# highlando/dolfin_navier_scipy

Measured on NVIDIA B200. Metric: cylinder-wake DoF*steps/s, higher is better.
Workload: dtype f64

## Files before the change

dolfin_navier_scipy_b200/csrc/dnsb_api.cu:

```cuda
#include "../../include/dnsb.h"

#include <algorithm>
#include <cmath>
#include <cstdlib>
#include <cstring>
#include <ctime>
#include <new>

#include "dnsb_common.cuh"
#include <cuda.h>
#ifdef DNSB_NO_NC
#define __restrict__
#endif
#include "dnsb_kernels.cuh"
#include "dnsb_batched.cuh"
#include "dnsb_dense.cuh"
#include "dnsb_stream.cuh"
#include "dnsb_tc.cuh"
#include "dnsb_tile.cuh"

#define DNSB_VERSION 100

#define LAUNCH(ctx, kern, grid, block, smem, ...)                              \
  do {                                                                         \
// ... 307 lines not shown
  DNSB_CK(ctx, m->t_runs.upload(runs.data(), runs.size(), ctx->stream));
  DNSB_CK(ctx, m->t_pidx.upload(pidx.data(), pidx.size(), ctx->stream));
  DNSB_CK(ctx, m->t_pval.upload(pval.data(), pval.size(), ctx->stream));
  {
    std::vector<float> pvalf(pval.size());
    std::vector<int> pidxf(pidx.size());
    for (size_t q = 0; q < pval.size(); ++q) pvalf[q] = (float)pval[q];
    for (size_t q = 0; q < pidx.size(); ++q) pidxf[q] = pidx[q] / 2;
    DNSB_CK(ctx, m->t_pvalf.upload(pvalf.data(), pvalf.size(), ctx->stream));
    DNSB_CK(ctx, m->t_pidxf.upload(pidxf.data(), pidxf.size(), ctx->stream));
  }
  p.ok = true;
  return 0;
}

static void csr_free(dnsb_csr *m) {
  if (!m) return;
  m->t_uptr.release(); m->t_rptr.release(); m->t_runs.release(); m->t_pidx.release(); m->t_pval.release();
  m->t_pidxf.release(); m->t_pvalf.release(); m->t_truns.release(); m->t_tdesc.release(); m->t_pdesc.release();
  m->indptr.release(); m->indices.release(); m->v1.release(); m->v2.release();
  delete m;
}

static inline bool batched_ok(const dnsb_csr *A, int nb) {
  return nb > 1 && (size_t)std::max(A->ncols, A->nrows) * nb < ((size_t)1 << 31);
}

static int g_rows_per_cta = 4;
static int g_dense_ctas_per_sm = 2;
static int g_graphs = 1;
static int g_schur_tf32 = 0;
static int g_dmma = 1;
static int g_schur_l2keep = 0;
static int g_tc_ctas = 1;
static int g_schur_tc = 1;
static const int TC_SMEM_OPTIN = 208 * 1024;
static int g_conv_colours = 0;
static inline int spb_gpc(dnsb_ctx *ctx, int nrows, int nb) {
  const long total = (long)nrows * nb;
  long gpc = std::max<long>(1, ((long)g_rows_per_cta * nb) / SPB_THREADS);
  const long groups = (total + SPB_THREADS - 1) / SPB_THREADS;
  while (gpc > 1 && (groups + gpc - 1) / gpc < 2L * ctx->sm_count) gpc /= 2;
  return (int)gpc;
}
static int g_pair = 1;
static inline bool pair_ok(const dnsb_csr *A, int nb) {
  return g_pair && batched_ok(A, nb) && nb % 2 == 0;
}
static inline unsigned spb2_grid(int nrows, int nb) {
  return cdiv((size_t)nrows * (nb / 2), SPB_THREADS);
}
static int g_rowpair = 1;
static inline int rowpairs_of(const dnsb_csr *A, int nb) {
  return (g_rowpair && pair_ok(A, nb)) ? A->npair_rows / 2 : 0;
}
static inline unsigned spp_grid(int npairs, int nb) {
  return cdiv((size_t)npairs * (nb / 2), SPB_THREADS);
}
#define D2C(p) reinterpret_cast<const double2 *>(p)
#define D2(p) reinterpret_cast<double2 *>(p)
static inline unsigned spb_grid(int nrows, int nb, int gpc) {
  return cdiv((size_t)nrows * nb, (size_t)SPB_THREADS * gpc);
}

static int g_tma_min_rows = 65536;
static inline bool spt_ok(const dnsb_csr *A, int nb) {
  return nb == 1 && A->spt.stages >= 2 && A->nrows >= g_tma_min_rows;
// ... 82 lines not shown
    const size_t threads = (size_t)A->nrows * nb;
    LAUNCH(ctx, k_spmm<1>, cdiv(threads, 256), 256, 0, A->view(), coef, x, z, y,
           nb, alpha, beta);
  }
}

static void fill_tabulation(double phi[7][6], double dphi[7][6][3], double qw[7], double lam[7][3]) {
  const double s15 = std::sqrt(15.0);
  const double a1 = (6.0 - s15) / 21.0, a2 = (6.0 + s15) / 21.0;
  const double w1 = (155.0 - s15) / 1200.0, w2 = (155.0 + s15) / 1200.0;
  const double qp[7][3] = {{1. / 3, 1. / 3, 1. / 3},
                           {1 - 2 * a1, a1, a1}, {a1, 1 - 2 * a1, a1}, {a1, a1, 1 - 2 * a1},
                           {1 - 2 * a2, a2, a2}, {a2, 1 - 2 * a2, a2}, {a2, a2, 1 - 2 * a2}};
  const double w[7] = {9. / 40, w1, w1, w1, w2, w2, w2};
  for (int q = 0; q < 7; ++q) {
    const double l0 = qp[q][0], l1 = qp[q][1], l2 = qp[q][2];
    qw[q] = w[q];
    lam[q][0] = l0; lam[q][1] = l1; lam[q][2] = l2;
    phi[q][0] = l0 * (2 * l0 - 1); phi[q][1] = l1 * (2 * l1 - 1);
    phi[q][2] = l2 * (2 * l2 - 1); phi[q][3] = 4 * l1 * l2;
    phi[q][4] = 4 * l0 * l2;       phi[q][5] = 4 * l0 * l1;
    for (int a = 0; a < 6; ++a)
      for (int i = 0; i < 3; ++i) dphi[q][a][i] = 0.0;
    dphi[q][0][0] = 4 * l0 - 1; dphi[q][1][1] = 4 * l1 - 1; dphi[q][2][2] = 4 * l2 - 1;
    dphi[q][3][1] = 4 * l2; dphi[q][3][2] = 4 * l1;
    dphi[q][4][0] = 4 * l2; dphi[q][4][2] = 4 * l0;
    dphi[q][5][0] = 4 * l1; dphi[q][5][1] = 4 * l0;
  }
}

#define DNSB_SWITCH_LIST(X) X(g_rows_per_cta) X(g_pair) X(g_tma_min_rows) X(g_gs_tma) X(g_tma_rows) X(g_tma_stages) \
  X(g_dmma) X(g_schur_tf32) X(g_schur_tc) X(g_tile) X(g_gs_pyth) X(g_schur_l2keep) X(g_tile_stages)             \
  X(g_tile_stages_f) X(g_tail_warps) X(g_pkeep) X(g_proj_t) X(g_cheb_f32) X(g_conv_colours) X(g_rowpair)         \
  X(g_graphs) X(g_dense_ctas_per_sm) X(g_tilef_ctas) X(g_tc_ctas) X(g_init_tile)
static void switches_store(int *sw) {
  int k = 0;
#define X(name) sw[k++] = name;
  DNSB_SWITCH_LIST(X)
#undef X
}
static void switches_load(const int *sw) {
  int k = 0;
#define X(name) name = sw[k++];
  DNSB_SWITCH_LIST(X)
#undef X
}
static const dnsb_ctx *g_switch_owner = nullptr;
static inline cudaError_t dnsb_enter(const dnsb_ctx *ctx) {
  if (g_switch_owner != ctx) { switches_load(ctx->sw); g_switch_owner = ctx; }
  return cudaSetDevice(ctx->device);
}

extern "C" int dnsb_version(void) { return DNSB_VERSION; }

extern "C" int dnsb_ctx_create(int device, dnsb_ctx **out) {
  if (!out) return -2;
  *out = nullptr;
  dnsb_ctx *ctx = new (std::nothrow) dnsb_ctx();
  if (!ctx) return -3;
  ctx->device = device;
  {
    static int defaults[32];
    static bool have_defaults = false;
    if (!have_defaults) { switches_store(defaults); have_defaults = true; }
    switches_load(defaults);
  }
  if (const char *ev = getenv("DNSB_ROWS_PER_CTA")) g_rows_per_cta = std::max(1, atoi(ev));
  if (const char *ev = getenv("DNSB_PAIR")) g_pair = atoi(ev);
  if (const char *ev = getenv("DNSB_TMA_MIN_ROWS")) g_tma_min_rows = atoi(ev);
  if (const char *ev = getenv("DNSB_GS_TMA")) g_gs_tma = atoi(ev);
  if (const char *ev = getenv("DNSB_TMA_ROWS")) g_tma_rows = std::min(SPT_ROWS, std::max(4, atoi(ev) & ~3));
  if (const char *ev = getenv("DNSB_TMA_STAGES")) g_tma_stages = std::min(SPT_MAX_STAGES, std::max(2, atoi(ev)));
  if (const char *ev = getenv("DNSB_DMMA")) g_dmma = atoi(ev);
  if (const char *ev = getenv("DNSB_SCHUR_TF32")) g_schur_tf32 = atoi(ev);
  if (const char *ev = getenv("DNSB_SCHUR_TC")) g_schur_tc = atoi(ev);
  if (const char *ev = getenv("DNSB_TILE")) g_tile = atoi(ev);
  if (const char *ev = getenv("DNSB_GS_PYTH")) g_gs_pyth = atoi(ev);
  if (const char *ev = getenv("DNSB_INIT_TILE")) g_init_tile = atoi(ev);
  if (const char *ev = getenv("DNSB_TC_CTAS")) g_tc_ctas = atoi(ev);
  if (const char *ev = getenv("DNSB_TILEF_CTAS")) g_tilef_ctas = atoi(ev);
  if (const char *ev = getenv("DNSB_PDL")) ctx->pdl = atoi(ev);
  if (const char *ev = getenv("DNSB_PDL_ONLY")) ctx->pdl_only = ev;
  if (const char *ev = getenv("DNSB_PDL_SKIP")) ctx->pdl_skip = ev;
  if (const char *ev = getenv("DNSB_SCHUR_L2KEEP")) g_schur_l2keep = atoi(ev);
  if (const char *ev = getenv("DNSB_TILE_STAGES")) g_tile_stages = std::max(2, std::min(TILE_MAX_STAGES, atoi(ev)));
  if (const char *ev = getenv("DNSB_TILE_STAGES_F")) g_tile_stages_f = std::max(2, std::min(TILE_MAX_STAGES, atoi(ev)));
  if (const char *ev = getenv("DNSB_TAIL_WARPS")) g_tail_warps = std::max(0, std::min(TILE_TAIL_WARPS_MAX, atoi(ev)));
  if (const char *ev = getenv("DNSB_PKEEP")) g_pkeep = atoi(ev);
  if (const char *ev = getenv("DNSB_PROJ_T")) g_proj_t = atoi(ev);
  if (const char *ev = getenv("DNSB_CHEB_F32")) g_cheb_f32 = atoi(ev);
  if (const char *ev = getenv("DNSB_CONV_COLOURS")) g_conv_colours = atoi(ev);
  if (const char *ev = getenv("DNSB_ROWPAIR")) g_rowpair = atoi(ev);
  if (const char *ev = getenv("DNSB_GRAPHS")) g_graphs = atoi(ev);
  if (const char *ev = getenv("DNSB_DENSE_CTAS_PER_SM")) g_dense_ctas_per_sm = std::max(1, atoi(ev));
  switches_store(ctx->sw);
  g_switch_owner = ctx;
  *out = ctx;
  DNSB_CK(ctx, cudaSetDevice(device));
  cudaDeviceProp prop;
  DNSB_CK(ctx, cudaGetDeviceProperties(&prop, device));
  ctx->sm_count = prop.multiProcessorCount;
  ctx->cc = prop.major * 10 + prop.minor;
  ctx->mem_bytes = prop.totalGlobalMem;
  DNSB_CK(ctx, cudaStreamCreateWithFlags(&ctx->stream, cudaStreamNonBlocking));
  double phi[7][6], dphi[7][6][3], qw[7], lam[7][3];
  fill_tabulation(phi, dphi, qw, lam);
  DNSB_CK(ctx, cudaMemcpyToSymbol(c_phi, phi, sizeof phi));
  DNSB_CK(ctx, cudaMemcpyToSymbol(c_dphi, dphi, sizeof dphi));
  DNSB_CK(ctx, cudaMemcpyToSymbol(c_qw, qw, sizeof qw));
  DNSB_CK(ctx, cudaMemcpyToSymbol(c_lam, lam, sizeof lam));
  DNSB_CK(ctx, cudaFuncSetAttribute(k_mdot_b, cudaFuncAttributeMaxDynamicSharedMemorySize, 200 * 1024));
  DNSB_CK(ctx, cudaFuncSetAttribute(k_gs_tma<false>, cudaFuncAttributeMaxDynamicSharedMemorySize, 112 * 1024));
// ... 610 lines not shown
  DNSB_CK(ctx, s->gg.alloc((size_t)(mr + 1) * nb));
  DNSB_CK(ctx, s->gh.alloc((size_t)(mr + 2) * nb));
  DNSB_CK(ctx, s->gh2.alloc((size_t)(mr + 2) * nb));
  DNSB_CK(ctx, s->ginvh.alloc(nb));
  DNSB_CK(ctx, s->gbnorm.alloc(nb));
  DNSB_CK(ctx, s->gresid.alloc(nb));
  DNSB_CK(ctx, s->gdone.alloc(nb));
  DNSB_CK(ctx, s->gits.alloc(nb));
  DNSB_CK(ctx, s->gittot.alloc(nb));
  DNSB_CK(ctx, s->gflags.alloc(4));
  DNSB_CK(ctx, s->grelmax.alloc(nb));
  DNSB_CK(ctx, s->grelmax.zero(ctx->stream));
  s->gs.R = s->gR.p; s->gs.cs = s->gcs.p; s->gs.sn = s->gsn.p; s->gs.g = s->gg.p;
  s->gs.h = s->gh.p; s->gs.invh = s->ginvh.p; s->gs.bnorm = s->gbnorm.p;
  s->gs.resid = s->gresid.p; s->gs.done = s->gdone.p; s->gs.its = s->gits.p;
  s->gs.ittot = s->gittot.p; s->gs.flags = s->gflags.p; s->gs.relmax = s->grelmax.p; s->gs.mr = mr;
  DNSB_CK(ctx, cudaMallocHost((void **)&s->h_flags, 4 * sizeof(int)));
  DNSB_CK(ctx, cudaStreamSynchronize(ctx->stream));
  DNSB_CK(ctx, cudaGetLastError());
  return 0;
}

static void dense_split(dnsb_ctx *ctx, int n, int nb, int *tn, DenseSplit *sp) {
  *tn = nb <= 16 ? 16 : (nb <= 32 ? 32 : 64);
  const int rt = cdiv(n, DGK_TM);
  sp->ksteps = cdiv(n, DGK_TK);
  const long units = (long)rt * sp->ksteps;
  long P = std::min<long>(units, (long)g_dense_ctas_per_sm * ctx->sm_count);
  sp->upc = (int)((units + P - 1) / P);
  sp->nctas = (int)((units + sp->upc - 1) / sp->upc);
  sp->maxseg = 2 + sp->upc / sp->ksteps;
}

typedef CUresult (*dnsb_encode_tiled_fn)(CUtensorMap *, CUtensorMapDataType, cuuint32_t, void *,
                                         const cuuint64_t *, const cuuint64_t *, const cuuint32_t *,
                                         const cuuint32_t *, CUtensorMapInterleave, CUtensorMapSwizzle,
                                         CUtensorMapL2promotion, CUtensorMapFloatOOBfill);
static dnsb_encode_tiled_fn tc_encode_fn() {
  static dnsb_encode_tiled_fn fn = nullptr;
  if (!fn) {
    void *p = nullptr;
    cudaDriverEntryPointQueryResult q;
    if (cudaGetDriverEntryPoint("cuTensorMapEncodeTiled", &p, cudaEnableDefault, &q) == cudaSuccess &&
        q == cudaDriverEntryPointSuccess)
      fn = (dnsb_encode_tiled_fn)p;
  }
  return fn;
}
static bool tc_map_2d(CUtensorMap *map, const float *base, int rows, int cols, int ld, int box_rows) {
  dnsb_encode_tiled_fn enc = tc_encode_fn();
  if (!enc) return false;
  const cuuint64_t gdim[2] = {(cuuint64_t)cols, (cuuint64_t)rows};
  const cuuint64_t gstride[1] = {(cuuint64_t)ld * sizeof(float)};
  const cuuint32_t box[2] = {TC_BK, (cuuint32_t)box_rows};
  const cuuint32_t estr[2] = {1, 1};
  return enc(map, CU_TENSOR_MAP_DATA_TYPE_FLOAT32, 2, (void *)base, gdim, gstride, box, estr,
             CU_TENSOR_MAP_INTERLEAVE_NONE, CU_TENSOR_MAP_SWIZZLE_128B, CU_TENSOR_MAP_L2_PROMOTION_L2_256B,
             CU_TENSOR_MAP_FLOAT_OOB_FILL_NONE) == CUDA_SUCCESS;
}
static cudaError_t tc_setup(dnsb_ctx *ctx, MgLevel *L, int n, int nb) {
  TcPlan &p = L->tc;
  p.ok = false;
  if (ctx->cc < 100 || nb < 8 || nb > 256 || n < TC_BM) return cudaSuccess;
  p.np_ = (nb + 15) & ~15;
  p.kblocks = (n + TC_BK - 1) / TC_BK;
  p.mtiles = (n + TC_BM - 1) / TC_BM;
  const int per_sm = std::max(1, std::min(2, g_tc_ctas));
  p.splits = std::max(1, std::min(p.kblocks, per_sm * ctx->sm_count / p.mtiles));
  p.kb_per_split = (p.kblocks + p.splits - 1) / p.splits;
  p.splits = (p.kblocks + p.kb_per_split - 1) / p.kb_per_split;
  const size_t a_bytes = (size_t)TC_BM * TC_BK * 4;
  const size_t b_bytes = (((size_t)p.np_ * TC_BK * 4) + 1023) & ~(size_t)1023;
  p.stages = (int)std::min<size_t>(TC_MAX_STAGES, ((size_t)TC_SMEM_OPTIN / per_sm - 1024) / (a_bytes + b_bytes));
  if (p.stages < 2) return cudaSuccess;
  p.smem = (size_t)p.stages * (a_bytes + b_bytes) + 1024;
  p.ldx = (n + 3) & ~3;
  cudaError_t e;
  if ((e = L->xt.alloc((size_t)p.np_ * p.ldx)) != cudaSuccess) return e;
  if ((e = L->xt.zero(ctx->stream)) != cudaSuccess) return e;
  if ((e = L->tcpart.alloc((size_t)p.splits * p.mtiles * TC_BM * p.np_)) != cudaSuccess) return e;
  if ((e = L->dinv_f32.alloc((size_t)p.mtiles * p.kblocks * TC_BM * TC_BK)) != cudaSuccess) return e;
  LAUNCH(ctx, k_tc_pack_d, cdiv(L->dinv_f32.n, 256), 256, 0, (const double *)L->dinv_dense.p, L->dinv_f32.p, n,
         p.mtiles, p.kblocks);
  p.ok = tc_map_2d(&p.mapB, L->xt.p, p.np_, n, p.ldx, p.np_);
  return cudaSuccess;
}

static void level_free(MgLevel *L) {
  if (!L) return;
  L->dinv_dense.release(); L->gpart.release(); L->dinv_f32.release(); L->x_f32.release(); L->xt.release(); L->tcpart.release(); L->dinv_own.release(); L->b.release(); L->x.release();
  L->r.release(); L->d0.release(); L->d1.release(); L->t.release();
  delete L;
}

extern "C" void dnsb_solver_destroy(dnsb_solver *s) {
  if (!s) return;
  dnsb_enter(s->ctx);
  const bool trace = getenv("DNSB_TRACE_DESTROY") != nullptr;
  auto now = [] { timespec ts; clock_gettime(CLOCK_MONOTONIC, &ts); return ts.tv_sec + 1e-9 * ts.tv_nsec; };
  double t0 = now();
  auto lap = [&](const char *what) { if (trace) { double t = now(); fprintf(stderr, "[destroy] %-12s %.2f ms\n", what, 1e3 * (t - t0)); t0 = t; } };
  cudaStreamSynchronize(s->ctx->stream);
  lap("sync");
  for (cudaGraphExec_t g : s->igraph) if (g) cudaGraphExecDestroy(g);
  s->igraph.clear();
  lap("graphs");
  csr_free(s->K);
  lap("K");
  s->coef.release(); s->dinv.release(); s->diagpos.release();
  s->Vb.release(); s->Zb.release(); s->w.release();
  lap("bases");
  s->cf_res.release(); s->cf_d0.release(); s->cf_d1.release(); s->cf_z.release(); s->cf_dinv.release();
  s->cres.release(); s->cd0.release(); s->cd1.release();
  s->partial.release(); s->partial2.release(); s->red.release();
  s->gR.release(); s->gcs.release(); s->gsn.release(); s->gg.release(); s->gh.release(); s->gh2.release();
  s->ginvh.release(); s->gbnorm.release(); s->gresid.release(); s->grelmax.release();
  s->gdone.release(); s->gits.release(); s->gittot.release(); s->gflags.release();
// ... 123 lines not shown
  dnsb_ctx *ctx = s->ctx;
  DNSB_REQUIRE(ctx, mp_dinv && mp_scale, "null arguments");
  DNSB_CK(ctx, dnsb_enter(ctx));
  DNSB_CK(ctx, s->mp_dinv.upload(mp_dinv, s->np, ctx->stream));
  DNSB_CK(ctx, s->mp_scale.upload(mp_scale, s->nb, ctx->stream));
  s->has_mass = true;
  solver_drop_graphs(s);
  return 0;
}

extern "C" int dnsb_solver_set_schur_lsc(dnsb_solver *s, const double *du_inv) {
  if (!s) return -2;
  dnsb_ctx *ctx = s->ctx;
  DNSB_REQUIRE(ctx, du_inv != nullptr, "null argument");
  DNSB_REQUIRE(ctx, !s->levels.empty(), "add the levels of L = J Du^-1 JT first");
  DNSB_CK(ctx, dnsb_enter(ctx));
  const size_t nvb = (size_t)s->nv * s->nb, npb = (size_t)s->np * s->nb;
  DNSB_CK(ctx, s->lsc_dinv.upload(du_inv, s->nv, ctx->stream));
  DNSB_CK(ctx, s->lsc_t1.alloc(nvb)); DNSB_CK(ctx, s->lsc_t2.alloc(nvb));
  DNSB_CK(ctx, s->lsc_p1.alloc(npb)); DNSB_CK(ctx, s->lsc_p2.alloc(npb));
  s->has_lsc = true;
  solver_drop_graphs(s);
  return 0;
}

static int dense_apply(dnsb_solver *s, MgLevel *L, const double *x,
                       double *y, double alpha, bool with_mass) {
  dnsb_ctx *ctx = s->ctx;
  const int n = L->n, nb = s->nb;
  const double *ad = with_mass ? s->mp_dinv.p : nullptr;
  const double *as = with_mass ? s->mp_scale.p : nullptr;
  if (L->tc.ok) {
    const TcPlan &p = L->tc;
    int tmem_cols = 32;
    while (tmem_cols < p.np_) tmem_cols *= 2;
    LAUNCH(ctx, k_tc_pack_x, dim3(cdiv(p.ldx, 32), cdiv(nb, 32)), 256, 0, x, L->xt.p, n, nb, p.ldx);
    LAUNCH(ctx, k_schur_tc, dim3(p.mtiles, p.splits), TC_THREADS, p.smem, (const float *)L->dinv_f32.p, p.mapB, L->tcpart.p, p.np_,
           p.kblocks, p.kb_per_split, p.stages, tmem_cols, g_schur_l2keep);
    LAUNCH(ctx, k_tc_epilogue, cdiv((size_t)n * nb, 256), 256, 0, (const float *)L->tcpart.p, p.splits,
           (size_t)p.mtiles * TC_BM * p.np_, p.np_, x, y, n, nb, alpha, ad, as);
    return 0;
  }
  if (nb <= 1)
    LAUNCH(ctx, k_dense_gemv<1>, cdiv((size_t)n * 32, 256), 256, 0, L->dinv_dense.p, x, y, n, nb, alpha, ad, as);
  else if (nb <= 2)
    LAUNCH(ctx, k_dense_gemv<2>, cdiv((size_t)n * 32, 256), 256, 0, L->dinv_dense.p, x, y, n, nb, alpha, ad, as);
  else if (nb <= 4)
    LAUNCH(ctx, k_dense_gemv<4>, cdiv((size_t)n * 32, 256), 256, 0, L->dinv_dense.p, x, y, n, nb, alpha, ad, as);
  else if (nb <= 8)
    LAUNCH(ctx, k_dense_gemv<8>, cdiv((size_t)n * 32, 256), 256, 0, L->dinv_dense.p, x, y, n, nb, alpha, ad, as);
  else {
    int tn;
    DenseSplit sp;
    dense_split(ctx, n, nb, &tn, &sp);
    const dim3 grid(sp.nctas, cdiv(nb, tn));
    if (g_schur_tf32 && L->dinv_f32.p && L->x_f32.p && tn == 64) {
      LAUNCH(ctx, k_f64_to_f32, cdiv((size_t)n * nb, 256), 256, 0, x, L->x_f32.p, (size_t)n, (size_t)nb, (size_t)nb);
const float *df_ = L->dinv_f32.p, *xf_ = L->x_f32.p;
      if (g_schur_tf32 == 1)
        LAUNCH(ctx, k_dense_tf32_streamk<3>, grid, 128, TFM_SMEM_BYTES, df_, L->ldf, xf_, L->gpart.p, n, nb, sp);
      else if (g_schur_tf32 == 2)
        LAUNCH(ctx, k_dense_tf32_streamk<2>, grid, 128, TFM_SMEM_BYTES, df_, L->ldf, xf_, L->gpart.p, n, nb, sp);
      else
        LAUNCH(ctx, k_dense_tf32_streamk<1>, grid, 128, TFM_SMEM_BYTES, df_, L->ldf, xf_, L->gpart.p, n, nb, sp);
    } else if (g_dmma && nb > 32 && n % 2 == 0 && nb % 2 == 0)
      LAUNCH(ctx, k_dense_dmma_streamk, grid, 128, DMM_SMEM_BYTES, L->dinv_dense.p, x, L->gpart.p, n, nb, sp);
    else if (tn == 16)
      LAUNCH(ctx, k_dense_gemm_streamk<16>, grid, 128, 0, L->dinv_dense.p, x, L->gpart.p, n, nb, sp);
    else if (tn == 32)
      LAUNCH(ctx, k_dense_gemm_streamk<32>, grid, 128, 0, L->dinv_dense.p, x, L->gpart.p, n, nb, sp);
    else
      LAUNCH(ctx, k_dense_gemm_streamk<64>, grid, 128, 0, L->dinv_dense.p, x, L->gpart.p, n, nb, sp);
    LAUNCH(ctx, k_dense_epilogue, cdiv((size_t)n * nb, 256), 256, 0, (const double *)L->gpart.p, sp, x,
// ... 1919 lines not shown
```

dolfin_navier_scipy_b200/csrc/dnsb_tc.cuh:

```cuda
#pragma once
#include <cuda.h>
#include <cuda_runtime.h>
#include <cstdint>

#define TC_BM 128
#define TC_BK 32
#define TC_UK 8
#define TC_THREADS 192
#define TC_MAX_STAGES 8

struct TcPlan {
  CUtensorMap mapB;
  int np_ = 0;
  int mtiles = 0, splits = 0, kblocks = 0, kb_per_split = 0, stages = 0;
  int ldx = 0;
  size_t smem = 0;
  bool ok = false;
};

__device__ __forceinline__ uint32_t tc_smem(const void *p) {
  return (uint32_t)__cvta_generic_to_shared(p);
}
__device__ __forceinline__ void tc_mbar_init(uint64_t *b, uint32_t count) {
  asm volatile("mbarrier.init.shared::cta.b64 [%0], %1;" ::"r"(tc_smem(b)), "r"(count) : "memory");
}
__device__ __forceinline__ void tc_mbar_expect(uint64_t *b, uint32_t bytes) {
  asm volatile("mbarrier.arrive.expect_tx.shared::cta.b64 _, [%0], %1;" ::"r"(tc_smem(b)), "r"(bytes)
               : "memory");
}
__device__ __forceinline__ void tc_mbar_wait(uint64_t *b, uint32_t parity) {
  const uint32_t a = tc_smem(b);
  uint32_t ok;
  do {
    asm volatile(
        "{\n\t.reg .pred p;\n\t"
        "mbarrier.try_wait.parity.shared::cta.b64 p, [%1], %2;\n\t"
        "selp.u32 %0, 1, 0, p;\n\t}"
        : "=r"(ok)
        : "r"(a), "r"(parity)
        : "memory");
  } while (!ok);
}
__device__ __forceinline__ void tc_tma_2d(void *dst, const CUtensorMap *map, int c0, int c1, uint64_t *bar) {
  asm volatile(
      "cp.async.bulk.tensor.2d.shared::cluster.global.mbarrier::complete_tx::bytes [%0], [%1, {%2, %3}], [%4];"
      ::"r"(tc_smem(dst)), "l"(map), "r"(c0), "r"(c1), "r"(tc_smem(bar))
      : "memory");
}
__device__ __forceinline__ uint64_t tc_desc(uint32_t saddr) {
  uint64_t d = 0;
  d |= (uint64_t)((saddr >> 4) & 0x3FFF);
  d |= (uint64_t)1 << 16;
  d |= (uint64_t)(1024 >> 4) << 32;
  d |= (uint64_t)1 << 46;
  d |= (uint64_t)2 << 61;
  return d;
}
__device__ __forceinline__ void tc_mma_tf32(uint32_t tmem_d, uint64_t da, uint64_t db, uint32_t idesc,
                                            uint32_t accumulate) {
  asm volatile(
      "{\n\t.reg .pred p;\n\t"
      "setp.ne.b32 p, %4, 0;\n\t"
      "tcgen05.mma.cta_group::1.kind::tf32 [%0], %1, %2, %3, p;\n\t}"
      ::"r"(tmem_d), "l"(da), "l"(db), "r"(idesc), "r"(accumulate)
      : "memory");
}
__device__ __forceinline__ void tc_commit(uint64_t *bar) {
  asm volatile("tcgen05.commit.cta_group::1.mbarrier::arrive::one.shared::cluster.b64 [%0];" ::"r"(tc_smem(bar))
               : "memory");
}
__device__ __forceinline__ void tc_ld16(uint32_t taddr, uint32_t (&r)[16]) {
  asm volatile(
      "tcgen05.ld.sync.aligned.32x32b.x16.b32 "
      "{%0, %1, %2, %3, %4, %5, %6, %7, %8, %9, %10, %11, %12, %13, %14, %15}, [%16];"
      : "=r"(r[0]), "=r"(r[1]), "=r"(r[2]), "=r"(r[3]), "=r"(r[4]), "=r"(r[5]), "=r"(r[6]), "=r"(r[7]),
        "=r"(r[8]), "=r"(r[9]), "=r"(r[10]), "=r"(r[11]), "=r"(r[12]), "=r"(r[13]), "=r"(r[14]), "=r"(r[15])
      : "r"(taddr)
      : "memory");
}

__device__ __forceinline__ void tc_bulk_1d(void *dst, const void *src, uint32_t bytes, uint64_t *bar) {
  asm volatile("cp.async.bulk.shared::cluster.global.mbarrier::complete_tx::bytes [%0], [%1], %2, [%3];" ::"r"(
                   tc_smem(dst)),
               "l"(src), "r"(bytes), "r"(tc_smem(bar))
               : "memory");
}

__global__ void __launch_bounds__(TC_THREADS, 1)
k_schur_tc(const float *__restrict__ Dt, const __grid_constant__ CUtensorMap mapB,
           float *__restrict__ part, int NP, int kblocks, int kb_per_split, int stages, int tmem_cols,
           int l2keep) {
  extern __shared__ __align__(1024) unsigned char tc_raw[];
  __shared__ __align__(8) uint64_t full[TC_MAX_STAGES], empty[TC_MAX_STAGES], accum_full;
  __shared__ uint32_t tmem_base_s;
  unsigned char *ring = (unsigned char *)(((uintptr_t)tc_raw + 1023) & ~(uintptr_t)1023);
  const uint32_t a_bytes = TC_BM * TC_BK * 4, b_bytes = (uint32_t)NP * TC_BK * 4;
  const uint32_t stage_bytes = a_bytes + ((b_bytes + 1023) & ~1023u);
  const int warp = threadIdx.x >> 5, lane = threadIdx.x & 31;
  const int mtile = blockIdx.x, split = blockIdx.y;
  const int kb0 = split * kb_per_split, kb1 = min(kblocks, kb0 + kb_per_split);
  const int nkb = kb1 - kb0;

  if (threadIdx.x == 0) {
    for (int s = 0; s < stages; ++s) {
      tc_mbar_init(&full[s], 1);
      tc_mbar_init(&empty[s], 1);
    }
    tc_mbar_init(&accum_full, 1);
    asm volatile("fence.mbarrier_init.release.cluster;" ::: "memory");
    asm volatile("fence.proxy.async.shared::cta;" ::: "memory");
  }
  if (warp == 1) {
    asm volatile("tcgen05.alloc.cta_group::1.sync.aligned.shared::cta.b32 [%0], %1;" ::"r"(tc_smem(&tmem_base_s)),
                 "r"((uint32_t)tmem_cols)
                 : "memory");
    asm volatile("tcgen05.relinquish_alloc_permit.cta_group::1.sync.aligned;" ::: "memory");
  }
  asm volatile("tcgen05.fence::before_thread_sync;" ::: "memory");
  __syncthreads();
  asm volatile("tcgen05.fence::after_thread_sync;" ::: "memory");
  const uint32_t tmem_base = tmem_base_s;
  dnsb_pdl_entry();

  if (warp == 0) {
    if (lane == 0) {
      for (int i = 0; i < nkb; ++i) {
        const int s = i % stages;
        if (i >= stages) tc_mbar_wait(&empty[s], ((i / stages) - 1) & 1);
        unsigned char *st = ring + (size_t)s * stage_bytes;
        tc_mbar_expect(&full[s], a_bytes + b_bytes);
        tc_bulk_1d(st, Dt + ((size_t)mtile * kblocks + kb0 + i) * (TC_BM * TC_BK), a_bytes, &full[s]);
        tc_tma_2d(st + a_bytes, &mapB, (kb0 + i) * TC_BK, 0, &full[s]);
      }
    }
  } else if (warp == 1) {
    const uint32_t idesc = (1u << 4) | (2u << 7) | (2u << 10) | ((uint32_t)(NP >> 3) << 17) |
                           ((uint32_t)(TC_BM >> 4) << 24);
    for (int i = 0; i < nkb; ++i) {
      const int s = i % stages;
      tc_mbar_wait(&full[s], (i / stages) & 1);
      asm volatile("tcgen05.fence::after_thread_sync;" ::: "memory");
      if (lane == 0) {
        const uint32_t sa = tc_smem(ring + (size_t)s * stage_bytes), sb = sa + a_bytes;
        const uint64_t da = tc_desc(sa), db = tc_desc(sb);
#pragma unroll
        for (int k = 0; k < TC_BK / TC_UK; ++k)
          tc_mma_tf32(tmem_base, da + (uint64_t)(k * 2), db + (uint64_t)(k * 2), idesc, (i | k) != 0);
        tc_commit(&empty[s]);
        if (i == nkb - 1) tc_commit(&accum_full);
      }
      __syncwarp();
    }
  } else {
    const int q = warp & 3;
    const int row = mtile * TC_BM + q * 32 + lane;
    float *out = part + ((size_t)split * gridDim.x * TC_BM + row) * NP;
    if (nkb > 0) {
      tc_mbar_wait(&accum_full, 0);
      asm volatile("tcgen05.fence::after_thread_sync;" ::: "memory");
      for (int c = 0; c < NP; c += 16) {
        uint32_t r[16];
        tc_ld16(tmem_base + ((uint32_t)(q * 32) << 16) + (uint32_t)c, r);
        asm volatile("tcgen05.wait::ld.sync.aligned;" ::: "memory");
        float4 *o4 = reinterpret_cast<float4 *>(out + c);
#pragma unroll
        for (int v = 0; v < 4; ++v)
          o4[v] = make_float4(__uint_as_float(r[4 * v]), __uint_as_float(r[4 * v + 1]),
                              __uint_as_float(r[4 * v + 2]), __uint_as_float(r[4 * v + 3]));
      }
    } else {
      for (int c = 0; c < NP; ++c) out[c] = 0.0f;
    }
  }
  asm volatile("tcgen05.fence::before_thread_sync;" ::: "memory");
  __syncthreads();
  if (warp == 1)
    asm volatile("tcgen05.dealloc.cta_group::1.sync.aligned.b32 %0, %1;" ::"r"(tmem_base), "r"((uint32_t)tmem_cols)
                 : "memory");
}

__device__ __forceinline__ float tc_round_tf32(float v) {
  uint32_t r;
  asm("cvt.rna.tf32.f32 %0, %1;" : "=r"(r) : "f"(v));
  return __uint_as_float(r);
}

__global__ void k_tc_pack_d(const double *__restrict__ src, float *__restrict__ dst, int n, int mtiles,
                            int kblocks) {
  dnsb_pdl_entry();
  const size_t t = (size_t)blockIdx.x * blockDim.x + threadIdx.x;
  const size_t total = (size_t)mtiles * kblocks * TC_BM * TC_BK;
  if (t >= total) return;
  const int k = (int)(t & 31), r = (int)((t >> 5) & 127);
  const size_t tile = t >> 12;
  const int kb = (int)(tile % kblocks), mt = (int)(tile / kblocks);
  const int row = mt * TC_BM + r, col = kb * TC_BK + k;
  const float v = (row < n && col < n) ? tc_round_tf32((float)src[(size_t)row * n + col]) : 0.0f;
  dst[tile * (TC_BM * TC_BK) + (size_t)r * 32 + ((((k >> 2) ^ (r & 7)) << 2) | (k & 3))] = v;
}

__global__ void k_tc_pack_x(const double *__restrict__ x, float *__restrict__ xt, int n, int nb, int ldx) {
  dnsb_pdl_entry();
  __shared__ float tile[32][33];
  const int k0 = blockIdx.x * 32, m0 = blockIdx.y * 32;
  const int tx = threadIdx.x & 31, ty = threadIdx.x >> 5;
  for (int r = ty; r < 32; r += 8) {
    const int k = k0 + r, m = m0 + tx;
    tile[r][tx] = (k < n && m < nb) ? tc_round_tf32((float)x[(size_t)k * nb + m]) : 0.0f;
  }
  __syncthreads();
  for (int r = ty; r < 32; r += 8) {
    const int m = m0 + r, k = k0 + tx;
    if (m < nb && k < ldx) xt[(size_t)m * ldx + k] = tile[tx][r];
  }
}

__global__ void k_tc_epilogue(const float *__restrict__ part, int splits, size_t split_stride, int NP,
                              const double *__restrict__ x, double *__restrict__ y, int n, int nb,
                              double alpha, const double *__restrict__ add_dinv,
                              const double *__restrict__ add_scale) {
  dnsb_pdl_entry();
  const size_t t = (size_t)blockIdx.x * blockDim.x + threadIdx.x;
  if (t >= (size_t)n * nb) return;
  const int i = (int)(t / nb), m = (int)(t % nb);
  double v = 0.0;
  for (int s = 0; s < splits; ++s) v += (double)part[(size_t)s * split_stride + (size_t)i * NP + m];
  if (add_dinv) v += add_scale[m] * add_dinv[i] * x[t];
  y[t] = alpha * v;
}
```

Baseline: 1.771 billion.

## Stream-K split for tcgen05 Schur GEMM with double-buffered TMEM accumulators

Replaces the fixed split-K grid of the TF32 tcgen05 Schur-complement GEMM with a stream-K partition, so each CTA processes a contiguous range of (mtile, kblock) units across tile boundaries. The output is written to per-segment slots, and the epilogue reduces over exactly the slots covering each tile. Two TMEM accumulators let the MMA warp start the next segment while the store warps drain the previous one. The A-operand loads are issued before the PDL wait so they overlap the previous kernel. The B operand is now packed by a new kernel into swizzled per-kblock blocks loaded with 1D bulk copies, which drops the tensor-map TMA path. The cost is a more complex kernel, extra partial slots to reduce, and a grid-stride epilogue.

```diff
diff --git a/dolfin_navier_scipy_b200/csrc/dnsb_api.cu b/dolfin_navier_scipy_b200/csrc/dnsb_api.cu
--- a/dolfin_navier_scipy_b200/csrc/dnsb_api.cu
+++ b/dolfin_navier_scipy_b200/csrc/dnsb_api.cu
@@ -363,7 +363,8 @@
 static int g_schur_tf32 = 0;
 static int g_dmma = 1;
 static int g_schur_l2keep = 0;
-static int g_tc_ctas = 1;
+static int g_tc_ctas = 0;
+static int g_tc_streamk = 1;
 static int g_schur_tc = 1;
 static const int TC_SMEM_OPTIN = 208 * 1024;
 static int g_conv_colours = 0;
@@ -512,7 +513,7 @@
 #define DNSB_SWITCH_LIST(X) X(g_rows_per_cta) X(g_pair) X(g_tma_min_rows) X(g_gs_tma) X(g_tma_rows) X(g_tma_stages) \
   X(g_dmma) X(g_schur_tf32) X(g_schur_tc) X(g_tile) X(g_gs_pyth) X(g_schur_l2keep) X(g_tile_stages)             \
   X(g_tile_stages_f) X(g_tail_warps) X(g_pkeep) X(g_proj_t) X(g_cheb_f32) X(g_conv_colours) X(g_rowpair)         \
-  X(g_graphs) X(g_dense_ctas_per_sm) X(g_tilef_ctas) X(g_tc_ctas) X(g_init_tile)
+  X(g_graphs) X(g_dense_ctas_per_sm) X(g_tilef_ctas) X(g_tc_ctas) X(g_init_tile) X(g_tc_streamk)
 static void switches_store(int *sw) {
   int k = 0;
 #define X(name) sw[k++] = name;
@@ -558,6 +559,7 @@
   if (const char *ev = getenv("DNSB_GS_PYTH")) g_gs_pyth = atoi(ev);
   if (const char *ev = getenv("DNSB_INIT_TILE")) g_init_tile = atoi(ev);
   if (const char *ev = getenv("DNSB_TC_CTAS")) g_tc_ctas = atoi(ev);
+  if (const char *ev = getenv("DNSB_TC_STREAMK")) g_tc_streamk = atoi(ev);
   if (const char *ev = getenv("DNSB_TILEF_CTAS")) g_tilef_ctas = atoi(ev);
   if (const char *ev = getenv("DNSB_PDL")) ctx->pdl = atoi(ev);
   if (const char *ev = getenv("DNSB_PDL_ONLY")) ctx->pdl_only = ev;
@@ -1234,32 +1236,6 @@
   sp->maxseg = 2 + sp->upc / sp->ksteps;
 }
 
-typedef CUresult (*dnsb_encode_tiled_fn)(CUtensorMap *, CUtensorMapDataType, cuuint32_t, void *,
-                                         const cuuint64_t *, const cuuint64_t *, const cuuint32_t *,
-                                         const cuuint32_t *, CUtensorMapInterleave, CUtensorMapSwizzle,
-                                         CUtensorMapL2promotion, CUtensorMapFloatOOBfill);
-static dnsb_encode_tiled_fn tc_encode_fn() {
-  static dnsb_encode_tiled_fn fn = nullptr;
-  if (!fn) {
-    void *p = nullptr;
-    cudaDriverEntryPointQueryResult q;
-    if (cudaGetDriverEntryPoint("cuTensorMapEncodeTiled", &p, cudaEnableDefault, &q) == cudaSuccess &&
-        q == cudaDriverEntryPointSuccess)
-      fn = (dnsb_encode_tiled_fn)p;
-  }
-  return fn;
-}
-static bool tc_map_2d(CUtensorMap *map, const float *base, int rows, int cols, int ld, int box_rows) {
-  dnsb_encode_tiled_fn enc = tc_encode_fn();
-  if (!enc) return false;
-  const cuuint64_t gdim[2] = {(cuuint64_t)cols, (cuuint64_t)rows};
-  const cuuint64_t gstride[1] = {(cuuint64_t)ld * sizeof(float)};
-  const cuuint32_t box[2] = {TC_BK, (cuuint32_t)box_rows};
-  const cuuint32_t estr[2] = {1, 1};
-  return enc(map, CU_TENSOR_MAP_DATA_TYPE_FLOAT32, 2, (void *)base, gdim, gstride, box, estr,
-             CU_TENSOR_MAP_INTERLEAVE_NONE, CU_TENSOR_MAP_SWIZZLE_128B, CU_TENSOR_MAP_L2_PROMOTION_L2_256B,
-             CU_TENSOR_MAP_FLOAT_OOB_FILL_NONE) == CUDA_SUCCESS;
-}
 static cudaError_t tc_setup(dnsb_ctx *ctx, MgLevel *L, int n, int nb) {
   TcPlan &p = L->tc;
   p.ok = false;
@@ -1267,24 +1243,38 @@
   p.np_ = (nb + 15) & ~15;
   p.kblocks = (n + TC_BK - 1) / TC_BK;
   p.mtiles = (n + TC_BM - 1) / TC_BM;
-  const int per_sm = std::max(1, std::min(2, g_tc_ctas));
-  p.splits = std::max(1, std::min(p.kblocks, per_sm * ctx->sm_count / p.mtiles));
-  p.kb_per_split = (p.kblocks + p.splits - 1) / p.splits;
-  p.splits = (p.kblocks + p.kb_per_split - 1) / p.kb_per_split;
+  const int per_sm = g_tc_ctas > 0 ? std::min(2, g_tc_ctas) : (g_tc_streamk ? 2 : 1);
+  const long units = (long)p.mtiles * p.kblocks;
+  if (g_tc_streamk) {
+    const long P = std::min<long>(units, (long)per_sm * ctx->sm_count);
+    p.upc = (int)((units + P - 1) / P);
+    p.nctas = (int)((units + p.upc - 1) / p.upc);
+    p.slots = p.nctas + p.mtiles - 1;
+    p.splits = p.kb_per_split = 0;
+  } else {
+    p.upc = p.nctas = 0;
+    p.splits = std::max(1, std::min(p.kblocks, per_sm * ctx->sm_count / p.mtiles));
+    p.kb_per_split = (p.kblocks + p.splits - 1) / p.splits;
+    p.splits = (p.kblocks + p.kb_per_split - 1) / p.kb_per_split;
+    p.slots = p.splits * p.mtiles;
+  }
   const size_t a_bytes = (size_t)TC_BM * TC_BK * 4;
   const size_t b_bytes = (((size_t)p.np_ * TC_BK * 4) + 1023) & ~(size_t)1023;
   p.stages = (int)std::min<size_t>(TC_MAX_STAGES, ((size_t)TC_SMEM_OPTIN / per_sm - 1024) / (a_bytes + b_bytes));
   if (p.stages < 2) return cudaSuccess;
   p.smem = (size_t)p.stages * (a_bytes + b_bytes) + 1024;
-  p.ldx = (n + 3) & ~3;
+  p.acc_cols = 32;
+  while (p.acc_cols < p.np_) p.acc_cols *= 2;
+  p.nacc = (g_tc_streamk && 2 * p.acc_cols * per_sm <= 512) ? 2 : 1;
+  p.npre = g_tc_streamk ? p.stages : 0;
   cudaError_t e;
-  if ((e = L->xt.alloc((size_t)p.np_ * p.ldx)) != cudaSuccess) return e;
-  if ((e = L->xt.zero(ctx->stream)) != cudaSuccess) return e;
-  if ((e = L->tcpart.alloc((size_t)p.splits * p.mtiles * TC_BM * p.np_)) != cudaSuccess) return e;
+  if ((e = L->xt.alloc((size_t)p.kblocks * p.np_ * TC_BK)) != cudaSuccess) return e;
+  if ((e = L->tcpart.alloc((size_t)p.slots * TC_BM * p.np_)) != cudaSuccess) return e;
   if ((e = L->dinv_f32.alloc((size_t)p.mtiles * p.kblocks * TC_BM * TC_BK)) != cudaSuccess) return e;
   LAUNCH(ctx, k_tc_pack_d, cdiv(L->dinv_f32.n, 256), 256, 0, (const double *)L->dinv_dense.p, L->dinv_f32.p, n,
          p.mtiles, p.kblocks);
-  p.ok = tc_map_2d(&p.mapB, L->xt.p, p.np_, n, p.ldx, p.np_);
+  dnsb_pdl_break();
+  p.ok = true;
   return cudaSuccess;
 }
 
@@ -1474,13 +1464,15 @@
   const double *as = with_mass ? s->mp_scale.p : nullptr;
   if (L->tc.ok) {
     const TcPlan &p = L->tc;
-    int tmem_cols = 32;
-    while (tmem_cols < p.np_) tmem_cols *= 2;
-    LAUNCH(ctx, k_tc_pack_x, dim3(cdiv(p.ldx, 32), cdiv(nb, 32)), 256, 0, x, L->xt.p, n, nb, p.ldx);
-    LAUNCH(ctx, k_schur_tc, dim3(p.mtiles, p.splits), TC_THREADS, p.smem, (const float *)L->dinv_f32.p, p.mapB, L->tcpart.p, p.np_,
-           p.kblocks, p.kb_per_split, p.stages, tmem_cols, g_schur_l2keep);
-    LAUNCH(ctx, k_tc_epilogue, cdiv((size_t)n * nb, 256), 256, 0, (const float *)L->tcpart.p, p.splits,
-           (size_t)p.mtiles * TC_BM * p.np_, p.np_, x, y, n, nb, alpha, ad, as);
+    const dim3 grid = p.upc > 0 ? dim3(p.nctas) : dim3(p.mtiles, p.splits);
+    LAUNCH(ctx, k_tc_pack_x, p.kblocks, TC_BK * p.np_ / TC_PACK_PER_THREAD, (size_t)TC_BK * (p.np_ + 1) * sizeof(float), x,
+           L->xt.p, n, nb, p.np_);
+    LAUNCH(ctx, k_schur_tc, grid, TC_THREADS, p.smem, (const float *)L->dinv_f32.p, (const float *)L->xt.p,
+           L->tcpart.p, p.np_, p.kblocks, p.mtiles * p.kblocks, p.upc, p.kb_per_split, p.stages, p.acc_cols, p.nacc,
+           p.npre);
+    const unsigned eg = std::min<unsigned>(cdiv((size_t)n * nb, 256), 8u * ctx->sm_count);
+    LAUNCH(ctx, k_tc_epilogue, eg, 256, 0, (const float *)L->tcpart.p, p.np_, p.kblocks, p.mtiles, p.upc, p.splits,
+           x, y, n, nb, alpha, ad, as);
     return 0;
   }
   if (nb <= 1)
diff --git a/dolfin_navier_scipy_b200/csrc/dnsb_tc.cuh b/dolfin_navier_scipy_b200/csrc/dnsb_tc.cuh
--- a/dolfin_navier_scipy_b200/csrc/dnsb_tc.cuh
+++ b/dolfin_navier_scipy_b200/csrc/dnsb_tc.cuh
@@ -8,12 +8,15 @@
 #define TC_UK 8
 #define TC_THREADS 192
 #define TC_MAX_STAGES 8
+#define TC_MAX_ACC 2
 
 struct TcPlan {
-  CUtensorMap mapB;
   int np_ = 0;
-  int mtiles = 0, splits = 0, kblocks = 0, kb_per_split = 0, stages = 0;
-  int ldx = 0;
+  int mtiles = 0, kblocks = 0, stages = 0;
+  int upc = 0, nctas = 0;
+  int splits = 0, kb_per_split = 0;
+  int slots = 0;
+  int acc_cols = 0, nacc = 0, npre = 0;
   size_t smem = 0;
   bool ok = false;
 };
@@ -41,12 +44,6 @@
         : "memory");
   } while (!ok);
 }
-__device__ __forceinline__ void tc_tma_2d(void *dst, const CUtensorMap *map, int c0, int c1, uint64_t *bar) {
-  asm volatile(
-      "cp.async.bulk.tensor.2d.shared::cluster.global.mbarrier::complete_tx::bytes [%0], [%1, {%2, %3}], [%4];"
-      ::"r"(tc_smem(dst)), "l"(map), "r"(c0), "r"(c1), "r"(tc_smem(bar))
-      : "memory");
-}
 __device__ __forceinline__ uint64_t tc_desc(uint32_t saddr) {
   uint64_t d = 0;
   d |= (uint64_t)((saddr >> 4) & 0x3FFF);
@@ -65,6 +62,9 @@
       ::"r"(tmem_d), "l"(da), "l"(db), "r"(idesc), "r"(accumulate)
       : "memory");
 }
+__device__ __forceinline__ void tc_mbar_arrive(uint64_t *b) {
+  asm volatile("mbarrier.arrive.shared::cta.b64 _, [%0];" ::"r"(tc_smem(b)) : "memory");
+}
 __device__ __forceinline__ void tc_commit(uint64_t *bar) {
   asm volatile("tcgen05.commit.cta_group::1.mbarrier::arrive::one.shared::cluster.b64 [%0];" ::"r"(tc_smem(bar))
                : "memory");
@@ -87,32 +87,45 @@
 }
 
 __global__ void __launch_bounds__(TC_THREADS, 1)
-k_schur_tc(const float *__restrict__ Dt, const __grid_constant__ CUtensorMap mapB,
-           float *__restrict__ part, int NP, int kblocks, int kb_per_split, int stages, int tmem_cols,
-           int l2keep) {
+k_schur_tc(const float *__restrict__ Dt, const float *__restrict__ Xt, float *__restrict__ part, int NP,
+           int kblocks, int units, int upc, int kb_per_split, int stages, int acc_cols, int nacc, int npre) {
   extern __shared__ __align__(1024) unsigned char tc_raw[];
-  __shared__ __align__(8) uint64_t full[TC_MAX_STAGES], empty[TC_MAX_STAGES], accum_full;
+  __shared__ __align__(8) uint64_t full[TC_MAX_STAGES], empty[TC_MAX_STAGES];
+  __shared__ __align__(8) uint64_t acc_full[TC_MAX_ACC], acc_empty[TC_MAX_ACC];
   __shared__ uint32_t tmem_base_s;
   unsigned char *ring = (unsigned char *)(((uintptr_t)tc_raw + 1023) & ~(uintptr_t)1023);
   const uint32_t a_bytes = TC_BM * TC_BK * 4, b_bytes = (uint32_t)NP * TC_BK * 4;
   const uint32_t stage_bytes = a_bytes + ((b_bytes + 1023) & ~1023u);
   const int warp = threadIdx.x >> 5, lane = threadIdx.x & 31;
-  const int mtile = blockIdx.x, split = blockIdx.y;
-  const int kb0 = split * kb_per_split, kb1 = min(kblocks, kb0 + kb_per_split);
-  const int nkb = kb1 - kb0;
+  int u0, u1, slot0;
+  if (upc > 0) {
+    u0 = blockIdx.x * upc;
+    u1 = min(units, u0 + upc);
+    slot0 = blockIdx.x + u0 / kblocks;
+  } else {
+    const int mtile = blockIdx.x, split = blockIdx.y;
+    u0 = mtile * kblocks + min(kblocks, split * kb_per_split);
+    u1 = mtile * kblocks + min(kblocks, (split + 1) * kb_per_split);
+    slot0 = split * gridDim.x + mtile;
+  }
+  const int nu = u1 - u0;
+  const int nseg = nu > 0 ? (u1 - 1) / kblocks - u0 / kblocks + 1 : 0;
 
   if (threadIdx.x == 0) {
     for (int s = 0; s < stages; ++s) {
       tc_mbar_init(&full[s], 1);
       tc_mbar_init(&empty[s], 1);
     }
-    tc_mbar_init(&accum_full, 1);
+    for (int b = 0; b < nacc; ++b) {
+      tc_mbar_init(&acc_full[b], 1);
+      tc_mbar_init(&acc_empty[b], 4);
+    }
     asm volatile("fence.mbarrier_init.release.cluster;" ::: "memory");
     asm volatile("fence.proxy.async.shared::cta;" ::: "memory");
   }
   if (warp == 1) {
     asm volatile("tcgen05.alloc.cta_group::1.sync.aligned.shared::cta.b32 [%0], %1;" ::"r"(tc_smem(&tmem_base_s)),
-                 "r"((uint32_t)tmem_cols)
+                 "r"((uint32_t)(nacc * acc_cols))
                  : "memory");
     asm volatile("tcgen05.relinquish_alloc_permit.cta_group::1.sync.aligned;" ::: "memory");
   }
@@ -120,24 +133,39 @@
   __syncthreads();
   asm volatile("tcgen05.fence::after_thread_sync;" ::: "memory");
   const uint32_t tmem_base = tmem_base_s;
+  const int np_pre = min(npre, min(stages, nu));
+  if (warp == 0 && lane == 0)
+    for (int i = 0; i < np_pre; ++i) {
+      unsigned char *st = ring + (size_t)i * stage_bytes;
+      tc_mbar_expect(&full[i], a_bytes + b_bytes);
+      tc_bulk_1d(st, Dt + (size_t)(u0 + i) * (TC_BM * TC_BK), a_bytes, &full[i]);
+    }
   dnsb_pdl_entry();
 
   if (warp == 0) {
     if (lane == 0) {
-      for (int i = 0; i < nkb; ++i) {
-        const int s = i % stages;
-        if (i >= stages) tc_mbar_wait(&empty[s], ((i / stages) - 1) & 1);
+      for (int i = 0; i < nu; ++i) {
+        const int s = i % stages, kb = (u0 + i) % kblocks;
         unsigned char *st = ring + (size_t)s * stage_bytes;
-        tc_mbar_expect(&full[s], a_bytes + b_bytes);
-        tc_bulk_1d(st, Dt + ((size_t)mtile * kblocks + kb0 + i) * (TC_BM * TC_BK), a_bytes, &full[s]);
-        tc_tma_2d(st + a_bytes, &mapB, (kb0 + i) * TC_BK, 0, &full[s]);
+        if (i >= np_pre) {
+          if (i >= stages) tc_mbar_wait(&empty[s], ((i / stages) - 1) & 1);
+          tc_mbar_expect(&full[s], a_bytes + b_bytes);
+          tc_bulk_1d(st, Dt + (size_t)(u0 + i) * (TC_BM * TC_BK), a_bytes, &full[s]);
+        }
+        tc_bulk_1d(st + a_bytes, Xt + (size_t)kb * NP * TC_BK, b_bytes, &full[s]);
       }
     }
   } else if (warp == 1) {
     const uint32_t idesc = (1u << 4) | (2u << 7) | (2u << 10) | ((uint32_t)(NP >> 3) << 17) |
                            ((uint32_t)(TC_BM >> 4) << 24);
-    for (int i = 0; i < nkb; ++i) {
-      const int s = i % stages;
+    int seg = 0;
+    for (int i = 0; i < nu; ++i) {
+      const int s = i % stages, u = u0 + i;
+      const bool seg_first = i == 0 || u % kblocks == 0, seg_last = i == nu - 1 || (u + 1) % kblocks == 0;
+      const int b = seg % nacc;
+      if (seg_first && seg >= nacc) {
+        tc_mbar_wait(&acc_empty[b], ((seg / nacc) - 1) & 1);
+      }
       tc_mbar_wait(&full[s], (i / stages) & 1);
       asm volatile("tcgen05.fence::after_thread_sync;" ::: "memory");
       if (lane == 0) {
@@ -145,37 +173,46 @@
         const uint64_t da = tc_desc(sa), db = tc_desc(sb);
 #pragma unroll
         for (int k = 0; k < TC_BK / TC_UK; ++k)
-          tc_mma_tf32(tmem_base, da + (uint64_t)(k * 2), db + (uint64_t)(k * 2), idesc, (i | k) != 0);
+          tc_mma_tf32(tmem_base + (uint32_t)(b * acc_cols), da + (uint64_t)(k * 2), db + (uint64_t)(k * 2), idesc,
+                      (!seg_first || k != 0) ? 1u : 0u);
         tc_commit(&empty[s]);
-        if (i == nkb - 1) tc_commit(&accum_full);
+        if (seg_last) tc_commit(&acc_full[b]);
       }
       __syncwarp();
+      if (seg_last) ++seg;
     }
   } else {
     const int q = warp & 3;
-    const int row = mtile * TC_BM + q * 32 + lane;
-    float *out = part + ((size_t)split * gridDim.x * TC_BM + row) * NP;
-    if (nkb > 0) {
-      tc_mbar_wait(&accum_full, 0);
+    const int r = q * 32 + lane;
+    for (int j = 0; j < nseg; ++j) {
+      const int b = j % nacc;
+      float *out = part + ((size_t)(slot0 + j) * TC_BM + r) * NP;
+      tc_mbar_wait(&acc_full[b], (j / nacc) & 1);
       asm volatile("tcgen05.fence::after_thread_sync;" ::: "memory");
       for (int c = 0; c < NP; c += 16) {
-        uint32_t r[16];
-        tc_ld16(tmem_base + ((uint32_t)(q * 32) << 16) + (uint32_t)c, r);
+        uint32_t v[16];
+        tc_ld16(tmem_base + ((uint32_t)(q * 32) << 16) + (uint32_t)(b * acc_cols + c), v);
         asm volatile("tcgen05.wait::ld.sync.aligned;" ::: "memory");
         float4 *o4 = reinterpret_cast<float4 *>(out + c);
 #pragma unroll
-        for (int v = 0; v < 4; ++v)
-          o4[v] = make_float4(__uint_as_float(r[4 * v]), __uint_as_float(r[4 * v + 1]),
-                              __uint_as_float(r[4 * v + 2]), __uint_as_float(r[4 * v + 3]));
-      }
-    } else {
+        for (int t = 0; t < 4; ++t)
+          o4[t] = make_float4(__uint_as_float(v[4 * t]), __uint_as_float(v[4 * t + 1]),
+                              __uint_as_float(v[4 * t + 2]), __uint_as_float(v[4 * t + 3]));
+      }
+      asm volatile("tcgen05.fence::before_thread_sync;" ::: "memory");
+      __syncwarp();
+      if (lane == 0) tc_mbar_arrive(&acc_empty[b]);
+    }
+    if (nseg == 0) {
+      float *out = part + ((size_t)slot0 * TC_BM + r) * NP;
       for (int c = 0; c < NP; ++c) out[c] = 0.0f;
     }
   }
   asm volatile("tcgen05.fence::before_thread_sync;" ::: "memory");
   __syncthreads();
   if (warp == 1)
-    asm volatile("tcgen05.dealloc.cta_group::1.sync.aligned.b32 %0, %1;" ::"r"(tmem_base), "r"((uint32_t)tmem_cols)
+    asm volatile("tcgen05.dealloc.cta_group::1.sync.aligned.b32 %0, %1;" ::"r"(tmem_base),
+                 "r"((uint32_t)(nacc * acc_cols))
                  : "memory");
 }
 
@@ -199,32 +236,54 @@
   dst[tile * (TC_BM * TC_BK) + (size_t)r * 32 + ((((k >> 2) ^ (r & 7)) << 2) | (k & 3))] = v;
 }
 
-__global__ void k_tc_pack_x(const double *__restrict__ x, float *__restrict__ xt, int n, int nb, int ldx) {
-  dnsb_pdl_entry();
-  __shared__ float tile[32][33];
-  const int k0 = blockIdx.x * 32, m0 = blockIdx.y * 32;
-  const int tx = threadIdx.x & 31, ty = threadIdx.x >> 5;
-  for (int r = ty; r < 32; r += 8) {
-    const int k = k0 + r, m = m0 + tx;
-    tile[r][tx] = (k < n && m < nb) ? tc_round_tf32((float)x[(size_t)k * nb + m]) : 0.0f;
+#define TC_PACK_PER_THREAD 8
+__global__ void k_tc_pack_x(const double *__restrict__ x, float *__restrict__ xt, int n, int nb, int NP) {
+  dnsb_pdl_entry();
+  extern __shared__ float tc_xs[];
+  const int ld = NP + 1, k0 = blockIdx.x * TC_BK;
+  const int rows = min(TC_BK, n - k0);
+  float v[TC_PACK_PER_THREAD];
+#pragma unroll
+  for (int j = 0; j < TC_PACK_PER_THREAD; ++j) {
+    const int t = threadIdx.x + j * blockDim.x, k = t / NP, m = t - k * NP;
+    v[j] = (k < rows && m < nb) ? tc_round_tf32((float)x[(size_t)(k0 + k) * nb + m]) : 0.0f;
+  }
+#pragma unroll
+  for (int j = 0; j < TC_PACK_PER_THREAD; ++j) {
+    const int t = threadIdx.x + j * blockDim.x, k = t / NP;
+    tc_xs[k * ld + (t - k * NP)] = v[j];
   }
   __syncthreads();
-  for (int r = ty; r < 32; r += 8) {
-    const int m = m0 + r, k = k0 + tx;
-    if (m < nb && k < ldx) xt[(size_t)m * ldx + k] = tile[tx][r];
-  }
-}
-
-__global__ void k_tc_epilogue(const float *__restrict__ part, int splits, size_t split_stride, int NP,
-                              const double *__restrict__ x, double *__restrict__ y, int n, int nb,
+  float *dst = xt + (size_t)blockIdx.x * NP * TC_BK;
+#pragma unroll
+  for (int j = 0; j < TC_PACK_PER_THREAD; ++j) {
+    const int t = threadIdx.x + j * blockDim.x;
+    const int m = t >> 5, pos = t & 31;
+    const int k = (((pos >> 2) ^ (m & 7)) << 2) | (pos & 3);
+    dst[t] = tc_xs[k * ld + m];
+  }
+}
+
+__global__ void k_tc_epilogue(const float *__restrict__ part, int NP, int kblocks, int mtiles, int upc,
+                              int splits, const double *__restrict__ x, double *__restrict__ y, int n, int nb,
                               double alpha, const double *__restrict__ add_dinv,
                               const double *__restrict__ add_scale) {
   dnsb_pdl_entry();
-  const size_t t = (size_t)blockIdx.x * blockDim.x + threadIdx.x;
-  if (t >= (size_t)n * nb) return;
-  const int i = (int)(t / nb), m = (int)(t % nb);
-  double v = 0.0;
-  for (int s = 0; s < splits; ++s) v += (double)part[(size_t)s * split_stride + (size_t)i * NP + m];
-  if (add_dinv) v += add_scale[m] * add_dinv[i] * x[t];
-  y[t] = alpha * v;
-}
+  const size_t total = (size_t)n * nb, tile = (size_t)TC_BM * NP;
+  for (size_t t = (size_t)blockIdx.x * blockDim.x + threadIdx.x; t < total; t += (size_t)gridDim.x * blockDim.x) {
+    const int i = (int)(t / nb), m = (int)(t % nb);
+    const int mt = i / TC_BM;
+    const float *p = part + (size_t)(i - mt * TC_BM) * NP + m;
+    double v = 0.0;
+    if (upc > 0) {
+      const int c0 = (int)((long)mt * kblocks / upc), c1 = (int)(((long)mt * kblocks + kblocks - 1) / upc);
+#pragma unroll 4
+      for (int c = c0; c <= c1; ++c) v += (double)p[(size_t)(c + mt) * tile];
+    } else {
+#pragma unroll 4
+      for (int s = 0; s < splits; ++s) v += (double)p[(size_t)(s * mtiles + mt) * tile];
+    }
+    if (add_dinv) v += add_scale[m] * add_dinv[i] * x[t];
+    y[t] = alpha * v;
+  }
+}
```

Result: slower. 1.749 billion (median of 6 runs) (-1.3%).
